# INK-USC/RE-Net

Hardware: AMD Instinct MI355X
Metric: RGCN+GRU encoder triples/s at bs=1024 n_hidden=200 (full training step, both directions) (higher is better)
Workload: dtype f32; 1 GPU; ICEWS18-shaped synthetic stream (seed 999), n_hidden=200, seq_len=10, batch=1024 per GPU, dropout=0.50, fwd+bwd both directions + clip + Adam; parallelism=dp1, global_batch=1024, nodes=99312, edges=288792

## Files before the change

re-net_amd/csrc/gemm.hip:

```cpp
#include <cstdint>
#include <cstdlib>
#include <type_traits>
#include "common.h"

namespace {

constexpr int BM = 128, BN = 128, BK = 32;
constexpr int LDK = BK + 4;
constexpr int LDR = BM + 4;
constexpr int OPBUF = BM * LDK;
constexpr int THREADS = 256;
static_assert(BK * LDR <= OPBUF, "operand buffer too small");

typedef float f32x16 __attribute__((ext_vector_type(16)));

struct GemmArgs {
    const float* A;
    const float* B;
    float* C;
    const float* bias;
    int M, N, K, lda, ldb, ldc;
    float alpha, beta;
    int k_tiles_per_split;
    int split_k;
    float* partial;
    int xcd_order;
};

template <bool CONTIG_K>
__device__ __forceinline__ void load_tile(const float* __restrict__ P, int ld, int rows, int K, int row0,
                                          int k0, int tid, bool vec_ok, float4 (&r)[4]) {
#pragma unroll
    for (int i = 0; i < 4; ++i) {
        const int f = tid + THREADS * i;
        float4 v = make_float4(0.f, 0.f, 0.f, 0.f);
        if constexpr (CONTIG_K) {
            const int row = row0 + (f >> 3), k = k0 + ((f & 7) << 2);
            if (row < rows) {
                const float* p = P + (size_t)row * ld + k;
                if (vec_ok && k + 3 < K) v = *reinterpret_cast<const float4*>(p);
                else {
                    if (k < K) v.x = p[0];
                    if (k + 1 < K) v.y = p[1];
                    if (k + 2 < K) v.z = p[2];
                    if (k + 3 < K) v.w = p[3];
                }
            }
        } else {
            const int k = k0 + (f >> 5), row = row0 + ((f & 31) << 2);
            if (k < K) {
                const float* p = P + (size_t)k * ld + row;
                if (vec_ok && row + 3 < rows) v = *reinterpret_cast<const float4*>(p);
                else {
                    if (row < rows) v.x = p[0];
                    if (row + 1 < rows) v.y = p[1];
                    if (row + 2 < rows) v.z = p[2];
                    if (row + 3 < rows) v.w = p[3];
                }
            }
        }
        r[i] = v;
    }
}

__device__ __forceinline__ float4 shift_tail(float4 v, int d) {
    if (d == 1) return make_float4(v.y, v.z, v.w, 0.f);
    if (d == 2) return make_float4(v.z, v.w, 0.f, 0.f);
    return make_float4(v.w, 0.f, 0.f, 0.f);
}

template <bool CONTIG_K>
__device__ __forceinline__ void load_tile_any(const float* __restrict__ P, int ld, int rows, int K, int row0,
                                              int k0, int tid, bool small, float4 (&r)[4]) {
    if (small) {
        load_tile<CONTIG_K>(P, ld, rows, K, row0, k0, tid, false, r);
        return;
    }
#pragma unroll
    for (int i = 0; i < 4; ++i) {
        const int f = tid + THREADS * i;
        const int c = CONTIG_K ? k0 + ((f & 7) << 2) : row0 + ((f & 31) << 2);
        const int o = CONTIG_K ? row0 + (f >> 3) : k0 + (f >> 5);
        const int C = CONTIG_K ? K : rows;
        const int O = CONTIG_K ? rows : K;
        r[i] = *reinterpret_cast<const float4*>(P + (size_t)min(o, O - 1) * ld + min(c, C - 4));
    }
}

template <bool CONTIG_K>
__device__ __forceinline__ void store_tile(float* __restrict__ S, int rows, int K, int row0, int k0, int tid,
                                           bool small, const float4 (&r)[4]) {
#pragma unroll
    for (int i = 0; i < 4; ++i) {
        const int f = tid + THREADS * i;
        float4 v = r[i];
        if (!small) {
            const int c = CONTIG_K ? k0 + ((f & 7) << 2) : row0 + ((f & 31) << 2);
            const int o = CONTIG_K ? row0 + (f >> 3) : k0 + (f >> 5);
            const int C = CONTIG_K ? K : rows;
            const int O = CONTIG_K ? rows : K;
            if (o >= O || c >= C) v = make_float4(0.f, 0.f, 0.f, 0.f);
            else if (c > C - 4) v = shift_tail(v, c - (C - 4));
        }
        if constexpr (CONTIG_K) *reinterpret_cast<float4*>(&S[(f >> 3) * LDK + ((f & 7) << 2)]) = v;
        else *reinterpret_cast<float4*>(&S[(f >> 5) * LDR + ((f & 31) << 2)]) = v;
    }
}

template <bool CONTIG_K>
__device__ __forceinline__ float4 read_frag(const float* __restrict__ S, int row, int g, int ksel) {
    if constexpr (CONTIG_K) {
        return *reinterpret_cast<const float4*>(&S[row * LDK + 8 * g + 4 * ksel]);
    } else {
        const float* p = S + (8 * g + 4 * ksel) * LDR + row;
        return make_float4(p[0], p[LDR], p[2 * LDR], p[3 * LDR]);
    }
}

template <bool TA, bool TB>
__global__ __launch_bounds__(THREADS) void gemm_f32_generic_kernel(GemmArgs g) {
    __shared__ __attribute__((aligned(16))) float smem[2][2][OPBUF];
    const int tid = threadIdx.x;
    const int lane = tid & 63, wave = tid >> 6;
    const int wm = wave >> 1, wn = wave & 1;
    const int m0 = blockIdx.y * BM, n0 = blockIdx.x * BN;
    const int z = blockIdx.z;
    const int kt0 = z * g.k_tiles_per_split;
    const int kt_total = (g.K + BK - 1) / BK;
    const int kt1 = min(kt_total, kt0 + g.k_tiles_per_split);

    constexpr bool A_CK = !TA;
    constexpr bool B_CK = TB;
    const bool a_vec = ((g.lda & 3) == 0) && ((reinterpret_cast<uintptr_t>(g.A) & 15) == 0);
    const bool b_vec = ((g.ldb & 3) == 0) && ((reinterpret_cast<uintptr_t>(g.B) & 15) == 0);

    f32x16 acc[2][2];
#pragma unroll
    for (int i = 0; i < 2; ++i)
#pragma unroll
        for (int j = 0; j < 2; ++j)
#pragma unroll
            for (int r = 0; r < 16; ++r) acc[i][j][r] = 0.f;

    (void)a_vec; (void)b_vec;
    const bool a_full = (g.K < 4) || (g.M < 4);
    const bool b_full = (g.K < 4) || (g.N < 4);
    float4 ra[4], rb[4];
    if (kt0 < kt1) {
        load_tile_any<A_CK>(g.A, g.lda, g.M, g.K, m0, kt0 * BK, tid, a_full, ra);
        load_tile_any<B_CK>(g.B, g.ldb, g.N, g.K, n0, kt0 * BK, tid, b_full, rb);
        store_tile<A_CK>(smem[0][0], g.M, g.K, m0, kt0 * BK, tid, a_full, ra);
        store_tile<B_CK>(smem[0][1], g.N, g.K, n0, kt0 * BK, tid, b_full, rb);
        if (kt0 + 1 < kt1) {
            load_tile_any<A_CK>(g.A, g.lda, g.M, g.K, m0, (kt0 + 1) * BK, tid, a_full, ra);
            load_tile_any<B_CK>(g.B, g.ldb, g.N, g.K, n0, (kt0 + 1) * BK, tid, b_full, rb);
        }
    }
    __syncthreads();
    const int arow = wm * 64 + (lane & 31);
    const int brow = wn * 64 + (lane & 31);
    const int ksel = lane >> 5;

    for (int kt = kt0; kt < kt1; ++kt) {
        const int cur = (kt - kt0) & 1;
        if (kt + 1 < kt1) {
            store_tile<A_CK>(smem[cur ^ 1][0], g.M, g.K, m0, (kt + 1) * BK, tid, a_full, ra);
            store_tile<B_CK>(smem[cur ^ 1][1], g.N, g.K, n0, (kt + 1) * BK, tid, b_full, rb);
        }
        if (kt + 2 < kt1) {
            load_tile_any<A_CK>(g.A, g.lda, g.M, g.K, m0, (kt + 2) * BK, tid, a_full, ra);
            load_tile_any<B_CK>(g.B, g.ldb, g.N, g.K, n0, (kt + 2) * BK, tid, b_full, rb);
        }
        const float* As = smem[cur][0];
        const float* Bs = smem[cur][1];
#pragma unroll
        for (int kg = 0; kg < BK / 8; ++kg) {
            const float4 a0 = read_frag<A_CK>(As, arow, kg, ksel);
            const float4 a1 = read_frag<A_CK>(As, arow + 32, kg, ksel);
            const float4 b0 = read_frag<B_CK>(Bs, brow, kg, ksel);
            const float4 b1 = read_frag<B_CK>(Bs, brow + 32, kg, ksel);
            acc[0][0] = __builtin_amdgcn_mfma_f32_32x32x2f32(a0.x, b0.x, acc[0][0], 0, 0, 0);
            acc[0][1] = __builtin_amdgcn_mfma_f32_32x32x2f32(a0.x, b1.x, acc[0][1], 0, 0, 0);
            acc[1][0] = __builtin_amdgcn_mfma_f32_32x32x2f32(a1.x, b0.x, acc[1][0], 0, 0, 0);
            acc[1][1] = __builtin_amdgcn_mfma_f32_32x32x2f32(a1.x, b1.x, acc[1][1], 0, 0, 0);
            acc[0][0] = __builtin_amdgcn_mfma_f32_32x32x2f32(a0.y, b0.y, acc[0][0], 0, 0, 0);
            acc[0][1] = __builtin_amdgcn_mfma_f32_32x32x2f32(a0.y, b1.y, acc[0][1], 0, 0, 0);
            acc[1][0] = __builtin_amdgcn_mfma_f32_32x32x2f32(a1.y, b0.y, acc[1][0], 0, 0, 0);
            acc[1][1] = __builtin_amdgcn_mfma_f32_32x32x2f32(a1.y, b1.y, acc[1][1], 0, 0, 0);
            acc[0][0] = __builtin_amdgcn_mfma_f32_32x32x2f32(a0.z, b0.z, acc[0][0], 0, 0, 0);
            acc[0][1] = __builtin_amdgcn_mfma_f32_32x32x2f32(a0.z, b1.z, acc[0][1], 0, 0, 0);
            acc[1][0] = __builtin_amdgcn_mfma_f32_32x32x2f32(a1.z, b0.z, acc[1][0], 0, 0, 0);
            acc[1][1] = __builtin_amdgcn_mfma_f32_32x32x2f32(a1.z, b1.z, acc[1][1], 0, 0, 0);
            acc[0][0] = __builtin_amdgcn_mfma_f32_32x32x2f32(a0.w, b0.w, acc[0][0], 0, 0, 0);
            acc[0][1] = __builtin_amdgcn_mfma_f32_32x32x2f32(a0.w, b1.w, acc[0][1], 0, 0, 0);
            acc[1][0] = __builtin_amdgcn_mfma_f32_32x32x2f32(a1.w, b0.w, acc[1][0], 0, 0, 0);
            acc[1][1] = __builtin_amdgcn_mfma_f32_32x32x2f32(a1.w, b1.w, acc[1][1], 0, 0, 0);
        }
        __syncthreads();
    }

    const bool split = g.split_k > 1;
    float* Cout = split ? g.partial + (size_t)z * g.M * g.N : g.C;
    const int ldo = split ? g.N : g.ldc;
#pragma unroll
    for (int i = 0; i < 2; ++i)
#pragma unroll
        for (int j = 0; j < 2; ++j) {
            const int col = n0 + wn * 64 + j * 32 + (lane & 31);
            if (col >= g.N) continue;
            const float bv = (!split && g.bias) ? g.bias[col] : 0.f;
#pragma unroll
            for (int r = 0; r < 16; ++r) {
                const int row = m0 + wm * 64 + i * 32 + (r & 3) + 8 * (r >> 2) + 4 * ksel;
                if (row < g.M) {
                    float* p = Cout + (size_t)row * ldo + col;
                    if (split) *p = acc[i][j][r];
                    else {
                        float v = g.alpha * acc[i][j][r] + bv;
                        if (g.beta != 0.f) v += g.beta * (*p);
                        *p = v;
                    }
                }
            }
        }
}

typedef uint32_t u32x4 __attribute__((ext_vector_type(4)));

__device__ __forceinline__ void tile_of_block(int nbx, int nby, bool xcd_order, int& bx, int& by, int& bz) {
    bz = blockIdx.z;
    if (!xcd_order) { bx = blockIdx.x; by = blockIdx.y; return; }
    const int nb = nbx * nby;
    int t;
    if (gridDim.z == 1) {
        const int per = nb >> 3;
        const int L = blockIdx.x + nbx * blockIdx.y;
        t = L < 8 * per ? (L & 7) * per + (L >> 3) : L;
    } else {
        const int total = nb * (int)gridDim.z, per3 = total >> 3;
        const int L3 = blockIdx.x + nbx * (blockIdx.y + nby * blockIdx.z);
        const int v = L3 < 8 * per3 ? (L3 & 7) * per3 + (L3 >> 3) : L3;
        bz = v / nb;
        t = v - bz * nb;
    }
    const int ns = min(nbx, nby), nl = max(nbx, nby);
    const int w = min(ns, 8);
    const int p = t / (w * nl), r = t - p * (w * nl);
    const int wp = min(w, ns - p * w);
    const int l = r / wp, sh = p * w + (r - l * wp);
    if (nby <= nbx) { bx = l; by = sh; }
    else { by = l; bx = sh; }
}

template <bool CONTIG_K, int KT>
struct BufLoader {
    static constexpr int NI = KT / 8;
    static constexpr int CPR = KT / 4;
    static constexpr int LDKT = KT + 4;
    __amdgpu_buffer_rsrc_t rs;
    uint32_t off[NI];
    uint32_t kstep;
    int lim[NI];
    int rows, K;

    __device__ __forceinline__ void init(const float* P, int ld, int rows_, int K_, int row0, int tid) {
        rows = rows_; K = K_;
        const uint32_t extent = CONTIG_K ? (uint32_t)(rows - 1) * (uint32_t)ld + (uint32_t)K
                                         : (uint32_t)(K - 1) * (uint32_t)ld + (uint32_t)rows;
        rs = __builtin_amdgcn_make_buffer_rsrc(const_cast<float*>(P), (short)0, (int)(extent * 4u), 0x00020000);
        kstep = CONTIG_K ? (uint32_t)KT * 4u : (uint32_t)KT * (uint32_t)ld * 4u;
#pragma unroll
        for (int i = 0; i < NI; ++i) {
            const int f = tid + THREADS * i;
            if constexpr (CONTIG_K) {
                const int row = row0 + f / CPR, k = (f % CPR) << 2;
                off[i] = ((uint32_t)min(row, rows - 1) * (uint32_t)ld + (uint32_t)k) * 4u;
                lim[i] = k;
            } else {
                const int k = f >> 5, row = row0 + ((f & 31) << 2);
                off[i] = ((uint32_t)k * (uint32_t)ld + (uint32_t)min(row, rows - 1)) * 4u;
                lim[i] = 0;
            }
        }
    }

    __device__ __forceinline__ float4 load(int i, int kt) const {
        const u32x4 v = __builtin_amdgcn_raw_buffer_load_b128(rs, (int)(off[i] + (uint32_t)kt * kstep), 0, 0);
        return make_float4(__uint_as_float(v.x), __uint_as_float(v.y), __uint_as_float(v.z), __uint_as_float(v.w));
    }

    __device__ __forceinline__ float4 fix(int i, int k0, float4 v) const {
        if constexpr (CONTIG_K) {
            const int room = K - k0 - lim[i];
            v.x = room > 0 ? v.x : 0.f;
            v.y = room > 1 ? v.y : 0.f;
            v.z = room > 2 ? v.z : 0.f;
            v.w = room > 3 ? v.w : 0.f;
        }
        return v;
    }

    __device__ __forceinline__ void store(float* __restrict__ S, int i, int tid, float4 v) const {
        const int f = tid + THREADS * i;
        if constexpr (CONTIG_K) *reinterpret_cast<float4*>(&S[(f / CPR) * LDKT + ((f % CPR) << 2)]) = v;
        else *reinterpret_cast<float4*>(&S[(f >> 5) * LDR + ((f & 31) << 2)]) = v;
    }

    static __device__ __forceinline__ float4 frag(const float* __restrict__ S, int row, int g, int ksel) {
        if constexpr (CONTIG_K) {
            return *reinterpret_cast<const float4*>(&S[row * LDKT + 8 * g + 4 * ksel]);
        } else {
            const float* p = S + (8 * g + 4 * ksel) * LDR + row;
            return make_float4(p[0], p[LDR], p[2 * LDR], p[3 * LDR]);
        }
    }
};

template <int I, int N, class F>
__device__ __forceinline__ void static_for(F&& f) {
    if constexpr (I < N) {
        f(std::integral_constant<int, I>{});
        static_for<I + 1, N>(f);
    }
}

__device__ __forceinline__ float f4_get(const float4& v, int t) { return t == 0 ? v.x : t == 1 ? v.y : t == 2 ? v.z : v.w; }

__device__ __forceinline__ void store_acc(const GemmArgs& g, int m0, int n0, int z, int wm, int wn, int lane,
                                          const f32x16 (&acc)[2][2]) {
    const bool split = g.split_k > 1;
    float* Cout = split ? g.partial + (size_t)z * g.M * g.N : g.C;
    const int ldo = split ? g.N : g.ldc;
    const int half = lane >> 5;
    const bool accumulate = !split && g.beta != 0.f;
#pragma unroll
    for (int i = 0; i < 2; ++i)
#pragma unroll
        for (int j = 0; j < 2; ++j) {
            const int col = n0 + wn * 64 + j * 32 + (lane & 31);
            if (col >= g.N) continue;
            const float bv = (!split && g.bias) ? g.bias[col] : 0.f;
            const int row_base = m0 + wm * 64 + i * 32 + 4 * half;
            float old[16];
#pragma unroll
            for (int r = 0; r < 16; ++r) old[r] = 0.f;
            if (accumulate) {
#pragma unroll
                for (int r = 0; r < 16; ++r) {
                    const int row = min(row_base + (r & 3) + 8 * (r >> 2), g.M - 1);
                    old[r] = Cout[(size_t)row * ldo + col];
                }
            }
#pragma unroll
            for (int r = 0; r < 16; ++r) {
                const int row = row_base + (r & 3) + 8 * (r >> 2);
                if (row < g.M) {
                    float* p = Cout + (size_t)row * ldo + col;
                    if (split) *p = acc[i][j][r];
                    else *p = g.alpha * acc[i][j][r] + bv + (accumulate ? g.beta * old[r] : 0.f);
                }
            }
        }
}

#ifndef F32P_NOBAR
#define F32_LOOP_BARRIER() asm volatile("s_waitcnt lgkmcnt(0)\n\ts_barrier" ::: "memory")
#else
#define F32_LOOP_BARRIER() asm volatile("s_waitcnt lgkmcnt(0)" ::: "memory")
#endif

template <bool TA, bool TB, int KT, int WPE>
__global__ __launch_bounds__(THREADS, WPE) void gemm_f32_kernel(GemmArgs g) {
    constexpr bool A_CK = !TA;
    constexpr bool B_CK = TB;
    typedef BufLoader<A_CK, KT> LA;
    typedef BufLoader<B_CK, KT> LB;
    constexpr int NI = KT / 8, NG = KT / 8, NM = 16 * NG;
    constexpr int OPB = (BM * (KT + 4) > KT * LDR) ? BM * (KT + 4) : KT * LDR;
    __shared__ __attribute__((aligned(16))) float smem[2][2][OPB];
    const int tid = threadIdx.x;
    const int lane = tid & 63, wave = tid >> 6;
    const int wm = wave >> 1, wn = wave & 1;
    int bx, by, z;
    tile_of_block(gridDim.x, gridDim.y, g.xcd_order != 0, bx, by, z);
    const int m0 = by * BM, n0 = bx * BN;
    const int kt0 = z * g.k_tiles_per_split;
    const int kt_total = (g.K + KT - 1) / KT;
    const int kt1 = min(kt_total, kt0 + g.k_tiles_per_split);

    f32x16 acc[2][2];
#pragma unroll
    for (int i = 0; i < 2; ++i)
#pragma unroll
        for (int j = 0; j < 2; ++j)
#pragma unroll
            for (int r = 0; r < 16; ++r) acc[i][j][r] = 0.f;

    LA la;
    LB lb;
    la.init(g.A, g.lda, g.M, g.K, m0, tid);
    lb.init(g.B, g.ldb, g.N, g.K, n0, tid);
    float4 ra[NI], rb[NI];
#pragma unroll
    for (int i = 0; i < NI; ++i) { ra[i] = la.load(i, kt0); rb[i] = lb.load(i, kt0); }
#pragma unroll
    for (int i = 0; i < NI; ++i) {
        la.store(smem[0][0], i, tid, la.fix(i, kt0 * KT, ra[i]));
        lb.store(smem[0][1], i, tid, lb.fix(i, kt0 * KT, rb[i]));
    }
#pragma unroll
    for (int i = 0; i < NI; ++i) { ra[i] = la.load(i, kt0 + 1); rb[i] = lb.load(i, kt0 + 1); }
    asm volatile("s_waitcnt lgkmcnt(0)\n\ts_barrier" ::: "memory");

    const int arow = wm * 64 + (lane & 31);
    const int brow = wn * 64 + (lane & 31);
    const int ksel = lane >> 5;

    auto k_tile = [&](int kt, auto fixc) {
        constexpr bool FIX = decltype(fixc)::value;
        const int cur = (kt - kt0) & 1;
        const float* As = smem[cur][0];
        const float* Bs = smem[cur][1];
        float* An = smem[cur ^ 1][0];
        float* Bn = smem[cur ^ 1][1];
        float4 fa[2][2], fb[2][2];
        fa[0][0] = LA::frag(As, arow, 0, ksel);
        fb[0][0] = LB::frag(Bs, brow, 0, ksel);
        fa[0][1] = LA::frag(As, arow + 32, 0, ksel);
        fb[0][1] = LB::frag(Bs, brow + 32, 0, ksel);
        static_for<0, NM>([&](auto mc) {
            constexpr int m = mc.value, grp = m >> 4, t = (m >> 2) & 3, i = (m >> 1) & 1, j = m & 1, fbuf = grp & 1;
            acc[i][j] = __builtin_amdgcn_mfma_f32_32x32x2f32(f4_get(fa[fbuf][i], t), f4_get(fb[fbuf][j], t), acc[i][j],
                                                             0, 0, 0);
            __builtin_amdgcn_sched_barrier(0);
            if constexpr (grp + 1 < NG && (m & 15) < 4) {
                constexpr int q = m & 15;
                if constexpr (q == 0) fa[fbuf ^ 1][0] = LA::frag(As, arow, grp + 1, ksel);
                if constexpr (q == 1) fb[fbuf ^ 1][0] = LB::frag(Bs, brow, grp + 1, ksel);
                if constexpr (q == 2) fa[fbuf ^ 1][1] = LA::frag(As, arow + 32, grp + 1, ksel);
                if constexpr (q == 3) fb[fbuf ^ 1][1] = LB::frag(Bs, brow + 32, grp + 1, ksel);
            }
#ifndef F32P_NOSTAGE
            constexpr int STRIDE = (NM - 6) / (2 * NI);
            if constexpr (m >= 4 && (m - 4) % STRIDE == 0 && (m - 4) / STRIDE < 2 * NI) {
                constexpr int pc = (m - 4) / STRIDE, it = pc >> 1;
                if constexpr ((pc & 1) == 0) la.store(An, it, tid, FIX ? la.fix(it, (kt + 1) * KT, ra[it]) : ra[it]);
                else lb.store(Bn, it, tid, FIX ? lb.fix(it, (kt + 1) * KT, rb[it]) : rb[it]);
            }
            if constexpr (m >= 5 && (m - 5) % STRIDE == 0 && (m - 5) / STRIDE < 2 * NI) {
                constexpr int pc = (m - 5) / STRIDE, it = pc >> 1;
                if constexpr ((pc & 1) == 0) ra[it] = la.load(it, kt + 2);
                else rb[it] = lb.load(it, kt + 2);
            }
#endif
            __builtin_amdgcn_sched_barrier(0);
        });
        F32_LOOP_BARRIER();
    };
    const int kt_plain = min(kt1, kt_total - 2);
    int kt = kt0;
    for (; kt < kt_plain; ++kt) k_tile(kt, std::false_type{});
    for (; kt < kt1; ++kt) k_tile(kt, std::true_type{});
    store_acc(g, m0, n0, z, wm, wn, lane, acc);
}

__global__ __launch_bounds__(256) void splitk_reduce_kernel(const float* __restrict__ partial, int split_k,
                                                            int M, int N, float alpha, float beta,
                                                            const float* __restrict__ bias,
                                                            float* __restrict__ C, int ldc) {
    const size_t total = (size_t)M * N;
    for (size_t i = (size_t)blockIdx.x * blockDim.x + threadIdx.x; i < total;
         i += (size_t)gridDim.x * blockDim.x) {
        const int m = (int)(i / N), n = (int)(i % N);
        float s = 0.f;
        for (int z = 0; z < split_k; ++z) s += partial[(size_t)z * total + i];
        float v = alpha * s + (bias ? bias[n] : 0.f);
        float* p = C + (size_t)m * ldc + n;
        if (beta != 0.f) v += beta * (*p);
        *p = v;
    }
}

template <typename T>
__global__ __launch_bounds__(256) void colsum_kernel(const T* __restrict__ X, int M, int N, int ldx,
                                                     int rows_per_group, float beta, float* __restrict__ out) {
    __shared__ float red[4][64];
    const int lane = threadIdx.x & 63, wave = threadIdx.x >> 6;
    const int n = blockIdx.x * 64 + lane;
    const int g = blockIdx.y;
    const int m0 = g * rows_per_group, m1 = min(M, m0 + rows_per_group);
    float s0 = 0.f, s1 = 0.f, s2 = 0.f, s3 = 0.f;
    if (n < N) {
        int m = m0 + wave;
        for (; m + 12 < m1; m += 16) {
            s0 += (float)X[(size_t)m * ldx + n];
            s1 += (float)X[(size_t)(m + 4) * ldx + n];
            s2 += (float)X[(size_t)(m + 8) * ldx + n];
            s3 += (float)X[(size_t)(m + 12) * ldx + n];
        }
        for (; m < m1; m += 4) s0 += (float)X[(size_t)m * ldx + n];
    }
    red[wave][lane] = (s0 + s1) + (s2 + s3);
    __syncthreads();
    if (wave == 0 && n < N) {
        float r = (red[0][lane] + red[1][lane]) + (red[2][lane] + red[3][lane]);
        float* o = out + (size_t)g * N + n;
        if (beta != 0.f) r += beta * (*o);
        *o = r;
    }
}

__global__ __launch_bounds__(256) void scale_dev_kernel(float* __restrict__ x, size_t n,
                                                        const float* __restrict__ scale, float bound_in,
                                                        float* __restrict__ bound_out) {
    const float f = *scale;
    if (bound_out && blockIdx.x == 0 && threadIdx.x == 0) *bound_out = fabsf(f) * bound_in;
    if (f == 1.f) return;
    const size_t n4 = n >> 2;
    float4* x4 = reinterpret_cast<float4*>(x);
    for (size_t i = (size_t)blockIdx.x * blockDim.x + threadIdx.x; i < n4; i += (size_t)gridDim.x * blockDim.x) {
        float4 v = x4[i];
        x4[i] = make_float4(v.x * f, v.y * f, v.z * f, v.w * f);
    }
    if (blockIdx.x == 0 && threadIdx.x < (n & 3)) x[(n4 << 2) + threadIdx.x] *= f;
}

__global__ __launch_bounds__(256) void scale_dev_bf16_kernel(__bf16* __restrict__ x, size_t n,
                                                             const float* __restrict__ scale) {
    const float f = *scale;
    if (f == 1.f) return;
    for (size_t i = (size_t)blockIdx.x * blockDim.x + threadIdx.x; i < n; i += (size_t)gridDim.x * blockDim.x)
        x[i] = (__bf16)((float)x[i] * f);
}

inline int colsum_groups(int M) { return max(1, min(64, (M + 127) / 128)); }

template <typename T>
int colsum_impl(const T* X, int M, int N, int ldx, float* out, float beta, float* workspace,
                       size_t workspace_bytes, void* stream) {
    if (M < 0 || N <= 0 || ldx < N) return RENET_ERR_BADARG;
    const int G = colsum_groups(M);
    hipStream_t st = (hipStream_t)stream;
    if (G == 1) {
        RENET_LAUNCH((colsum_kernel<T>), dim3((N + 63) / 64, 1), dim3(256), 0, st, X, M, N, ldx, max(M, 1), beta, out);
        RENET_LAUNCH_CHECK();
        return RENET_OK;
    }
    if (workspace_bytes < (size_t)colsum_groups(M) * N * sizeof(float)) return RENET_ERR_WORKSPACE;
    const int rpg = (M + G - 1) / G;
    RENET_LAUNCH((colsum_kernel<T>), dim3((N + 63) / 64, G), dim3(256), 0, st, X, M, N, ldx, rpg, 0.f, workspace);
    RENET_LAUNCH_CHECK();
    RENET_LAUNCH((colsum_kernel<float>), dim3((N + 63) / 64, 1), dim3(256), 0, st, (const float*)workspace, G, N, N, G,
                 beta, out);
    RENET_LAUNCH_CHECK();
    return RENET_OK;
}


bool generic_forced() {
    static const bool v = renet_env_flag("RENET_GEMM_F32_GENERIC", false);
    return v;
}

}

extern "C" {

size_t renet_gemm_workspace(int M, int N, int split_k) {
    return split_k > 1 ? (size_t)split_k * (size_t)M * (size_t)N * sizeof(float) : 0;
}

int renet_gemm_f32(int ta, int tb, int M, int N, int K, float alpha, const float* A, int lda,
                   const float* B, int ldb, float beta, float* C, int ldc, const float* bias,
                   int split_k, float* workspace, size_t workspace_bytes, void* stream) {
    if (M < 0 || N < 0 || K < 0 || lda <= 0 || ldb <= 0 || ldc < N) return RENET_ERR_BADARG;
    if (M == 0 || N == 0) return RENET_OK;
    if (split_k < 1) split_k = 1;
    const int kt_total = (K + BK - 1) / BK;
    if (split_k > kt_total) split_k = max(kt_total, 1);
    if (split_k > 1 && workspace_bytes < renet_gemm_workspace(M, N, split_k)) return RENET_ERR_WORKSPACE;
    GemmArgs g;
    g.A = A; g.B = B; g.C = C; g.bias = bias; g.M = M; g.N = N; g.K = K;
    g.lda = lda; g.ldb = ldb; g.ldc = ldc; g.alpha = alpha; g.beta = beta;
    g.split_k = split_k;
    g.k_tiles_per_split = (kt_total + split_k - 1) / split_k;
    if (g.k_tiles_per_split < 1) g.k_tiles_per_split = 1;
    g.partial = workspace;
    g.xcd_order = renet_gemm_tile_order() != 0;
    hipStream_t st = (hipStream_t)stream;
    const dim3 grid((N + BN - 1) / BN, (M + BM - 1) / BM, split_k);
    const size_t reach_a = ta ? ((size_t)K + 3 * BK) * lda + M : (size_t)M * lda + K + 3 * BK;
    const size_t reach_b = tb ? (size_t)N * ldb + K + 3 * BK : ((size_t)K + 3 * BK) * ldb + N;
    const bool buffered = K >= 1 && reach_a < ((size_t)1 << 30) && reach_b < ((size_t)1 << 30) && !generic_forced();
    if (buffered) {
        constexpr int kt = 32;
        const int ktiles = (K + kt - 1) / kt;
        if (split_k > ktiles) { split_k = max(ktiles, 1); g.split_k = split_k; }
        g.k_tiles_per_split = max(1, (ktiles + split_k - 1) / split_k);
        const dim3 gridb((N + BN - 1) / BN, (M + BM - 1) / BM, split_k);
#define RENET_F32_LAUNCH(KT_, WPE_)                                                                                   \
        do {                                                                                                          \
            if (!ta && !tb) RENET_LAUNCH((gemm_f32_kernel<false, false, KT_, WPE_>), gridb, dim3(THREADS), 0, st, g); \
            else if (!ta && tb) RENET_LAUNCH((gemm_f32_kernel<false, true, KT_, WPE_>), gridb, dim3(THREADS), 0, st, g); \
            else if (ta && !tb) RENET_LAUNCH((gemm_f32_kernel<true, false, KT_, WPE_>), gridb, dim3(THREADS), 0, st, g); \
            else RENET_LAUNCH((gemm_f32_kernel<true, true, KT_, WPE_>), gridb, dim3(THREADS), 0, st, g);              \
        } while (0)
        RENET_F32_LAUNCH(32, 2);
#undef RENET_F32_LAUNCH
    } else {
        g.xcd_order = 0;
        if (!ta && !tb) RENET_LAUNCH((gemm_f32_generic_kernel<false, false>), grid, dim3(THREADS), 0, st, g);
        else if (!ta && tb) RENET_LAUNCH((gemm_f32_generic_kernel<false, true>), grid, dim3(THREADS), 0, st, g);
        else if (ta && !tb) RENET_LAUNCH((gemm_f32_generic_kernel<true, false>), grid, dim3(THREADS), 0, st, g);
        else RENET_LAUNCH((gemm_f32_generic_kernel<true, true>), grid, dim3(THREADS), 0, st, g);
    }
    RENET_LAUNCH_CHECK();
    if (split_k > 1) {
        const size_t total = (size_t)M * N;
        int blocks = (int)min((size_t)2048, (total + 255) / 256);
        RENET_LAUNCH(splitk_reduce_kernel, dim3(blocks), dim3(256), 0, st, workspace, split_k, M, N,
                           alpha, beta, bias, C, ldc);
        RENET_LAUNCH_CHECK();
    }
    return RENET_OK;
}

size_t renet_colsum_workspace(int M, int N) {
    const int G = colsum_groups(M);
    return G > 1 ? (size_t)G * (size_t)N * sizeof(float) : 0;
}

int renet_scale_by_device_scalar(float* x, size_t n, const float* scale, void* stream) {
    if (!x || !scale || (reinterpret_cast<uintptr_t>(x) & 15)) return RENET_ERR_BADARG;
    if (n == 0) return RENET_OK;
    const int blocks = (int)min((size_t)2048, (n / 4 + 255) / 256 + 1);
    RENET_LAUNCH(scale_dev_kernel, dim3(blocks), dim3(256), 0, (hipStream_t)stream, x, n, scale, 0.f, (float*)nullptr);
    RENET_LAUNCH_CHECK();
    return RENET_OK;
}

int renet_scale_by_device_scalar_bound(float* x, size_t n, const float* scale, float bound_in, float* bound_out,
                                       void* stream) {
    if (!x || !scale || !bound_out || (reinterpret_cast<uintptr_t>(x) & 15)) return RENET_ERR_BADARG;
    const int blocks = (int)min((size_t)2048, (n / 4 + 255) / 256 + 1);
    RENET_LAUNCH(scale_dev_kernel, dim3(blocks), dim3(256), 0, (hipStream_t)stream, x, n, scale, bound_in, bound_out);
    RENET_LAUNCH_CHECK();
    return RENET_OK;
}

int renet_colsum(const float* X, int M, int N, int ldx, float* out, float beta, float* workspace,
                 size_t workspace_bytes, void* stream) {
    return colsum_impl<float>(X, M, N, ldx, out, beta, workspace, workspace_bytes, stream);
}

int renet_colsum_bf16(const void* X, int M, int N, int ldx, float* out, float beta, float* workspace,
                      size_t workspace_bytes, void* stream) {
    return colsum_impl<__bf16>((const __bf16*)X, M, N, ldx, out, beta, workspace, workspace_bytes, stream);
}

int renet_scale_bf16_by_device_scalar(void* x, size_t n, const float* scale, void* stream) {
    if (n == 0) return RENET_OK;
    const int blocks = (int)min((size_t)2048, (n + 255) / 256);
    RENET_LAUNCH(scale_dev_bf16_kernel, dim3(blocks), dim3(256), 0, (hipStream_t)stream, (__bf16*)x, n, scale);
    RENET_LAUNCH_CHECK();
    return RENET_OK;
}

}
```

re-net_amd/csrc/rows.hip:

```cpp
#include "common.h"

namespace {

__global__ __launch_bounds__(256) void gather_rows_kernel(const float4* __restrict__ table,
                                                          const int32_t* __restrict__ idx, int n, int CH,
                                                          float4* __restrict__ out) {
    const size_t total = (size_t)n * CH;
    for (size_t i = (size_t)blockIdx.x * blockDim.x + threadIdx.x; i < total;
         i += (size_t)gridDim.x * blockDim.x) {
        const int r = (int)(i / CH), c = (int)(i % CH);
        out[i] = table[(size_t)idx[r] * CH + c];
    }
}

constexpr int kSegWaves = 16, kSegShort = 16, kSegUnr = 8;
__global__ __launch_bounds__(kSegWaves * 64) void segment_add_kernel(const float4* __restrict__ src0,
                                                                     const float4* __restrict__ src1,
                                                                     const int32_t* __restrict__ order,
                                                                     const int32_t* __restrict__ seg_ptr,
                                                                     const int32_t* __restrict__ seg_target,
                                                                     int U, int CH, float4* __restrict__ dst0,
                                                                     float4* __restrict__ dst1) {
    const float4* __restrict__ src = blockIdx.y ? src1 : src0;
    float4* __restrict__ dst = blockIdx.y ? dst1 : dst0;
    __shared__ float4 red[kSegWaves][128];
    const int lane = threadIdx.x & 63;
    const int wave = __builtin_amdgcn_readfirstlane(threadIdx.x >> 6);
    const int nwg = gridDim.x;
    {
        const int u = blockIdx.x + wave * nwg;
        const int k0 = u < U ? seg_ptr[u] : 0, k1 = u < U ? seg_ptr[u + 1] : 0;
        const int len = k1 - k0;
        if (len > 0 && len <= kSegShort) {
            const size_t tgt = (size_t)seg_target[u] * CH;
            for (int ch = lane; ch < CH; ch += 64) {
                float4 s = make_float4(0.f, 0.f, 0.f, 0.f);
                for (int k = k0; k < k1; k += kSegUnr) {
                    float4 v[kSegUnr];
#pragma unroll
                    for (int j = 0; j < kSegUnr; ++j) v[j] = src[(size_t)order[min(k + j, k1 - 1)] * CH + ch];
#pragma unroll
                    for (int j = 0; j < kSegUnr; ++j)
                        if (k + j < k1) s = f4_add(s, v[j]);
                }
                dst[tgt + ch] = f4_add(dst[tgt + ch], s);
            }
        }
    }
    for (int j = 0; j < kSegWaves; ++j) {
        const int u = blockIdx.x + j * nwg;
        if (u >= U) break;
        const int k0 = seg_ptr[u], k1 = seg_ptr[u + 1];
        if (k1 - k0 <= kSegShort) continue;
        const size_t tgt = (size_t)seg_target[u] * CH;
        for (int ch = lane; ch < CH; ch += 64) {
            float4 s = make_float4(0.f, 0.f, 0.f, 0.f);
            for (int k = k0 + wave * kSegUnr; k < k1; k += kSegWaves * kSegUnr) {
                float4 v[kSegUnr];
#pragma unroll
                for (int q = 0; q < kSegUnr; ++q) v[q] = src[(size_t)order[min(k + q, k1 - 1)] * CH + ch];
#pragma unroll
                for (int q = 0; q < kSegUnr; ++q)
                    if (k + q < k1) s = f4_add(s, v[q]);
            }
            red[wave][ch] = s;
        }
        __syncthreads();
        if (wave == 0) {
            for (int ch = lane; ch < CH; ch += 64) {
                float4 r = red[0][ch];
#pragma unroll
                for (int w = 1; w < kSegWaves; ++w) r = f4_add(r, red[w][ch]);
                dst[tgt + ch] = f4_add(dst[tgt + ch], r);
            }
        }
        __syncthreads();
    }
}

}

extern "C" {

int renet_version(void) { return RENET_ABI_VERSION; }

int renet_gather_rows(const float* table, const int32_t* idx, int n, int D, float* out, void* stream) {
    if (n < 0 || D <= 0 || (D & 3)) return RENET_ERR_BADARG;
    if (n == 0) return RENET_OK;
    const int CH = D / 4;
    const size_t total = (size_t)n * CH;
    int blocks = (int)min((size_t)2048, (total + 255) / 256);
    RENET_LAUNCH(gather_rows_kernel, dim3(blocks), dim3(256), 0, (hipStream_t)stream,
                       (const float4*)table, idx, n, CH, (float4*)out);
    RENET_LAUNCH_CHECK();
    return RENET_OK;
}

static int seg_grid(int U) { return U <= 512 ? U : max(512, (U + kSegWaves - 1) / kSegWaves); }

int renet_segment_add(const float* src, const int32_t* order, const int32_t* seg_ptr,
                      const int32_t* seg_target, int U, int D, float* dst, void* stream) {
    if (U < 0 || D <= 0 || (D & 3)) return RENET_ERR_BADARG;
    if (U == 0) return RENET_OK;
    if (D > 512) return RENET_ERR_UNSUPPORTED;
    RENET_LAUNCH(segment_add_kernel, dim3(seg_grid(U)), dim3(kSegWaves * 64), 0,
                       (hipStream_t)stream, (const float4*)src, (const float4*)src, order, seg_ptr, seg_target, U, D / 4,
                       (float4*)dst, (float4*)dst);
    RENET_LAUNCH_CHECK();
    return RENET_OK;
}

int renet_segment_add2(const float* src0, const float* src1, const int32_t* order, const int32_t* seg_ptr,
                       const int32_t* seg_target, int U, int D, float* dst0, float* dst1, void* stream) {
    if (U < 0 || D <= 0 || (D & 3)) return RENET_ERR_BADARG;
    if (U == 0) return RENET_OK;
    if (D > 512) return RENET_ERR_UNSUPPORTED;
    RENET_LAUNCH(segment_add_kernel, dim3(seg_grid(U), 2), dim3(kSegWaves * 64), 0,
                       (hipStream_t)stream, (const float4*)src0, (const float4*)src1, order, seg_ptr, seg_target, U, D / 4,
                       (float4*)dst0, (float4*)dst1);
    RENET_LAUNCH_CHECK();
    return RENET_OK;
}

}
```

Baseline: 391,300 triples/s.

## Restructure segment-add work split and vectorize column-sum kernel

Segment-add is reorganized into two kinds of workgroups in one launch. Some workgroups collect long segments and reduce each with 16 chains across 8 waves. The rest give one wave per short or medium segment, using readlane-broadcast indices, length-specialized unrolled gathers and software-prefetched segment bounds. The column-sum reduction also gains a float4-vectorized variant, used when stride and alignment allow. The aim is to cut load imbalance, index-load latency and per-element scalar loads in the scatter-add and bias-gradient paths, at the cost of more complex code and extra shared-memory atomics for classifying segments.

```diff
diff --git a/re-net_amd/csrc/gemm.hip b/re-net_amd/csrc/gemm.hip
--- a/re-net_amd/csrc/gemm.hip
+++ b/re-net_amd/csrc/gemm.hip
@@ -510,6 +510,70 @@
     }
 }
 
+constexpr int kColsumUnr = 8;
+template <typename T>
+__global__ __launch_bounds__(256) void colsum_vec_kernel(const T* __restrict__ X, int M, int N, int ldx,
+                                                         int rows_per_group, float beta, float* __restrict__ out) {
+    typedef T vec4 __attribute__((ext_vector_type(4)));
+    __shared__ float red[4][4][64];
+    const int lane = threadIdx.x & 63;
+    const int wave = __builtin_amdgcn_readfirstlane(threadIdx.x >> 6);
+    const int a = lane >> 4, n4 = blockIdx.x * 64 + (lane & 15) * 4;
+    const int g = blockIdx.y;
+    const int m0 = g * rows_per_group, m1 = min(M, m0 + rows_per_group);
+    const int b = m0 + wave;
+    const int I = m1 - 12 > b ? (m1 - 12 - b + 15) >> 4 : 0;
+    const int bt = b + 16 * I;
+    float s[4] = {0.f, 0.f, 0.f, 0.f};
+    if (n4 + 3 < N) {
+        const T* col = X + n4;
+        for (int i = 0; i < I; i += kColsumUnr) {
+            vec4 v[kColsumUnr];
+#pragma unroll
+            for (int j = 0; j < kColsumUnr; ++j)
+                v[j] = *reinterpret_cast<const vec4*>(col + (size_t)(b + 4 * a + 16 * min(i + j, I - 1)) * ldx);
+#pragma unroll
+            for (int j = 0; j < kColsumUnr; ++j) {
+                const bool on = i + j < I;
+#pragma unroll
+                for (int c = 0; c < 4; ++c) s[c] = on ? s[c] + (float)v[j][c] : s[c];
+            }
+        }
+        if (a == 0 && bt < m1) {
+            vec4 v[3];
+#pragma unroll
+            for (int j = 0; j < 3; ++j) v[j] = *reinterpret_cast<const vec4*>(col + (size_t)min(bt + 4 * j, m1 - 1) * ldx);
+#pragma unroll
+            for (int j = 0; j < 3; ++j) {
+                const bool on = bt + 4 * j < m1;
+#pragma unroll
+                for (int c = 0; c < 4; ++c) s[c] = on ? s[c] + (float)v[j][c] : s[c];
+            }
+        }
+    } else if (n4 < N) {
+        for (int i = 0; i < I; ++i)
+            for (int c = 0; c < 4; ++c)
+                if (n4 + c < N) s[c] += (float)X[(size_t)(b + 4 * a + 16 * i) * ldx + n4 + c];
+        if (a == 0)
+            for (int m = bt; m < m1; m += 4)
+                for (int c = 0; c < 4; ++c)
+                    if (n4 + c < N) s[c] += (float)X[(size_t)m * ldx + n4 + c];
+    }
+#pragma unroll
+    for (int c = 0; c < 4; ++c) red[wave][a][(lane & 15) * 4 + c] = s[c];
+    __syncthreads();
+    const int n = blockIdx.x * 64 + lane;
+    if (wave == 0 && n < N) {
+        float r[4];
+#pragma unroll
+        for (int w = 0; w < 4; ++w) r[w] = (red[w][0][lane] + red[w][1][lane]) + (red[w][2][lane] + red[w][3][lane]);
+        float t = (r[0] + r[1]) + (r[2] + r[3]);
+        float* o = out + (size_t)g * N + n;
+        if (beta != 0.f) t += beta * (*o);
+        *o = t;
+    }
+}
+
 __global__ __launch_bounds__(256) void scale_dev_kernel(float* __restrict__ x, size_t n,
                                                         const float* __restrict__ scale, float bound_in,
                                                         float* __restrict__ bound_out) {
@@ -536,22 +600,28 @@
 inline int colsum_groups(int M) { return max(1, min(64, (M + 127) / 128)); }
 
 template <typename T>
+void colsum_launch(const T* X, int M, int N, int ldx, int G, int rpg, float beta, float* out, hipStream_t st) {
+    const bool vec = (ldx & 3) == 0 && ((uintptr_t)X & (4 * sizeof(T) - 1)) == 0;
+    if (vec) RENET_LAUNCH((colsum_vec_kernel<T>), dim3((N + 63) / 64, G), dim3(256), 0, st, X, M, N, ldx, rpg, beta, out);
+    else RENET_LAUNCH((colsum_kernel<T>), dim3((N + 63) / 64, G), dim3(256), 0, st, X, M, N, ldx, rpg, beta, out);
+}
+
+template <typename T>
 int colsum_impl(const T* X, int M, int N, int ldx, float* out, float beta, float* workspace,
                        size_t workspace_bytes, void* stream) {
     if (M < 0 || N <= 0 || ldx < N) return RENET_ERR_BADARG;
     const int G = colsum_groups(M);
     hipStream_t st = (hipStream_t)stream;
     if (G == 1) {
-        RENET_LAUNCH((colsum_kernel<T>), dim3((N + 63) / 64, 1), dim3(256), 0, st, X, M, N, ldx, max(M, 1), beta, out);
+        colsum_launch<T>(X, M, N, ldx, 1, max(M, 1), beta, out, st);
         RENET_LAUNCH_CHECK();
         return RENET_OK;
     }
     if (workspace_bytes < (size_t)colsum_groups(M) * N * sizeof(float)) return RENET_ERR_WORKSPACE;
     const int rpg = (M + G - 1) / G;
-    RENET_LAUNCH((colsum_kernel<T>), dim3((N + 63) / 64, G), dim3(256), 0, st, X, M, N, ldx, rpg, 0.f, workspace);
+    colsum_launch<T>(X, M, N, ldx, G, rpg, 0.f, workspace, st);
     RENET_LAUNCH_CHECK();
-    RENET_LAUNCH((colsum_kernel<float>), dim3((N + 63) / 64, 1), dim3(256), 0, st, (const float*)workspace, G, N, N, G,
-                 beta, out);
+    colsum_launch<float>((const float*)workspace, G, N, N, 1, G, beta, out, st);
     RENET_LAUNCH_CHECK();
     return RENET_OK;
 }
diff --git a/re-net_amd/csrc/rows.hip b/re-net_amd/csrc/rows.hip
--- a/re-net_amd/csrc/rows.hip
+++ b/re-net_amd/csrc/rows.hip
@@ -13,68 +13,154 @@
     }
 }
 
-constexpr int kSegWaves = 16, kSegShort = 16, kSegUnr = 8;
-__global__ __launch_bounds__(kSegWaves * 64) void segment_add_kernel(const float4* __restrict__ src0,
-                                                                     const float4* __restrict__ src1,
-                                                                     const int32_t* __restrict__ order,
-                                                                     const int32_t* __restrict__ seg_ptr,
-                                                                     const int32_t* __restrict__ seg_target,
-                                                                     int U, int CH, float4* __restrict__ dst0,
-                                                                     float4* __restrict__ dst1) {
+constexpr int kSegShort = 16, kSegUnr = 8, kSegChains = 16, kSegMedium = kSegChains * kSegUnr, kSegWaves = 8;
+constexpr int kSegThreads = kSegWaves * 64, kSegMaxCH = 128;
+
+__device__ __forceinline__ float4 seg_sel(bool c, float4 a, float4 b) {
+    return make_float4(c ? a.x : b.x, c ? a.y : b.y, c ? a.z : b.z, c ? a.w : b.w);
+}
+
+template <int NR>
+__device__ __forceinline__ void seg_short_rows(const float4* __restrict__ src, float4* __restrict__ dst, int idx,
+                                               size_t tgt, int len, int CH, int lane) {
+    for (int c0 = 0; c0 < CH; c0 += 64) {
+        const int ch = c0 + lane, chc = min(ch, CH - 1);
+        float4 v[NR];
+#pragma unroll
+        for (int j = 0; j < NR; ++j) v[j] = src[(size_t)__builtin_amdgcn_readlane(idx, j) * CH + chc];
+        const float4 old = dst[tgt + chc];
+        float4 s = make_float4(0.f, 0.f, 0.f, 0.f);
+#pragma unroll
+        for (int j = 0; j < NR; ++j) s = seg_sel(j < len, f4_add(s, v[j]), s);
+        if (ch < CH) dst[tgt + ch] = f4_add(old, s);
+    }
+}
+
+__device__ __forceinline__ void seg_medium_rows(const float4* __restrict__ src, float4* __restrict__ dst,
+                                                const int32_t* __restrict__ order, int idx0, int k0, size_t tgt, int len,
+                                                int CH, int lane) {
+    const int idx1 = order[min(k0 + 64 + lane, k0 + len - 1)];
+    for (int c0 = 0; c0 < CH; c0 += 64) {
+        const int ch = c0 + lane, chc = min(ch, CH - 1);
+        const float4 old = dst[tgt + chc];
+        float4 r = make_float4(0.f, 0.f, 0.f, 0.f);
+        const float4 zero = make_float4(0.f, 0.f, 0.f, 0.f);
+        int b = 0;
+#pragma unroll 1
+        for (; 2 * kSegUnr * b < len; ++b) {
+            const int idx = b < 4 ? idx0 : idx1, l0 = (2 * kSegUnr * b) & 63;
+            float4 c[2], v[2 * kSegUnr];
+            c[0] = c[1] = zero;
+#pragma unroll
+            for (int q = 0; q < 2 * kSegUnr; ++q) v[q] = src[(size_t)__builtin_amdgcn_readlane(idx, l0 + q) * CH + chc];
+#pragma unroll
+            for (int q = 0; q < 2 * kSegUnr; ++q)
+                c[q / kSegUnr] = seg_sel(2 * kSegUnr * b + q < len, f4_add(c[q / kSegUnr], v[q]), c[q / kSegUnr]);
+            r = seg_sel(b == 0, c[0], f4_add(r, c[0]));
+            r = f4_add(r, c[1]);
+        }
+        for (; b < kSegChains / 2; ++b) r = f4_add(f4_add(r, zero), zero);
+        if (ch < CH) dst[tgt + ch] = f4_add(old, r);
+    }
+}
+
+__global__ __launch_bounds__(kSegThreads) __attribute__((amdgpu_waves_per_eu(2, 4))) void segment_add_kernel(
+    const float4* __restrict__ src0, const float4* __restrict__ src1, const int32_t* __restrict__ order,
+    const int32_t* __restrict__ seg_ptr, const int32_t* __restrict__ seg_target, int U, int CH, int n_long_wg,
+    float4* __restrict__ dst0, float4* __restrict__ dst1) {
     const float4* __restrict__ src = blockIdx.y ? src1 : src0;
     float4* __restrict__ dst = blockIdx.y ? dst1 : dst0;
-    __shared__ float4 red[kSegWaves][128];
-    const int lane = threadIdx.x & 63;
-    const int wave = __builtin_amdgcn_readfirstlane(threadIdx.x >> 6);
-    const int nwg = gridDim.x;
-    {
-        const int u = blockIdx.x + wave * nwg;
-        const int k0 = u < U ? seg_ptr[u] : 0, k1 = u < U ? seg_ptr[u + 1] : 0;
-        const int len = k1 - k0;
-        if (len > 0 && len <= kSegShort) {
-            const size_t tgt = (size_t)seg_target[u] * CH;
-            for (int ch = lane; ch < CH; ch += 64) {
-                float4 s = make_float4(0.f, 0.f, 0.f, 0.f);
-                for (int k = k0; k < k1; k += kSegUnr) {
-                    float4 v[kSegUnr];
-#pragma unroll
-                    for (int j = 0; j < kSegUnr; ++j) v[j] = src[(size_t)order[min(k + j, k1 - 1)] * CH + ch];
-#pragma unroll
-                    for (int j = 0; j < kSegUnr; ++j)
-                        if (k + j < k1) s = f4_add(s, v[j]);
+    __shared__ float4 red[kSegChains][kSegMaxCH];
+    __shared__ int list[kSegThreads];
+    __shared__ int cnt;
+    const int tid = threadIdx.x, lane = tid & 63;
+    const int wave = __builtin_amdgcn_readfirstlane(tid >> 6);
+
+    if ((int)blockIdx.x >= n_long_wg) {
+        const int gw = (blockIdx.x - n_long_wg) * kSegWaves + wave;
+        const int nw = (gridDim.x - n_long_wg) * kSegWaves;
+        const int R = seg_ptr[U];
+        if (R <= 0) return;
+        auto bound = [&](long long u, int& k0, int& k1) {
+            const int uc = (int)min(u, (long long)U - 1);
+            const int a = seg_ptr[uc], b = seg_ptr[uc + 1];
+            k0 = u < U ? a : 0;
+            k1 = u < U ? b : 0;
+        };
+        auto entries = [&](long long u, int k0, int len, int& idx, int& tgt) {
+            idx = order[min(k0 + min(lane, max(len - 1, 0)), R - 1)];
+            tgt = seg_target[(int)min(u, (long long)U - 1)];
+        };
+        long long u = gw;
+        int k0, k1, idx, tgt, nk0, nk1;
+        bound(u, k0, k1);
+        entries(u, k0, k1 - k0, idx, tgt);
+        bound(u + nw, nk0, nk1);
+        while (u < U) {
+            const int len = k1 - k0, nlen = nk1 - nk0;
+            int nidx, ntgt, nnk0, nnk1;
+            entries(u + nw, nk0, nlen, nidx, ntgt);
+            bound(u + 2ll * nw, nnk0, nnk1);
+            if (len > 0 && len <= kSegMedium) {
+                const size_t t = (size_t)tgt * CH;
+                if (len == 1) seg_short_rows<1>(src, dst, idx, t, len, CH, lane);
+                else if (len == 2) seg_short_rows<2>(src, dst, idx, t, len, CH, lane);
+                else if (len <= 4) seg_short_rows<4>(src, dst, idx, t, len, CH, lane);
+                else if (len <= 8) seg_short_rows<8>(src, dst, idx, t, len, CH, lane);
+                else if (len <= kSegShort) seg_short_rows<16>(src, dst, idx, t, len, CH, lane);
+                else seg_medium_rows(src, dst, order, idx, k0, t, len, CH, lane);
+            }
+            u += nw;
+            k0 = nk0, k1 = nk1, idx = nidx, tgt = ntgt, nk0 = nnk0, nk1 = nnk1;
+        }
+        return;
+    }
+
+    float* __restrict__ dstf = reinterpret_cast<float*>(dst);
+    const long long G = n_long_wg;
+    bool first = true;
+    for (long long base = 0; blockIdx.x + base * G < U; base += kSegThreads) {
+        __syncthreads();
+        if (tid == 0) cnt = 0;
+        __syncthreads();
+        const long long u = blockIdx.x + (base + tid) * G;
+        if (u < U && seg_ptr[u + 1] - seg_ptr[u] > kSegMedium) list[atomicAdd(&cnt, 1)] = (int)u;
+        __syncthreads();
+        const int n = cnt;
+        for (int i = 0; i < n; ++i) {
+            const int us = __builtin_amdgcn_readfirstlane(list[i]);
+            const int k0 = seg_ptr[us], k1 = seg_ptr[us + 1];
+            const size_t tgt = (size_t)seg_target[us] * CH * 4;
+            const float old = tid < 4 * CH ? dstf[tgt + tid] : 0.f;
+            if (!first) __syncthreads();
+            first = false;
+            for (int c0 = 0; c0 < CH; c0 += 64) {
+                const int ch = c0 + lane, chc = min(ch, CH - 1);
+                float4 s[2];
+                s[0] = s[1] = make_float4(0.f, 0.f, 0.f, 0.f);
+                int kb = k0 + 2 * kSegUnr * wave;
+                int idx = order[min(kb + (lane & 15), k1 - 1)];
+                for (; kb < k1; kb += kSegChains * kSegUnr) {
+                    const int idx_next = order[min(kb + kSegChains * kSegUnr + (lane & 15), k1 - 1)];
+                    float4 v[2 * kSegUnr];
+#pragma unroll
+                    for (int q = 0; q < 2 * kSegUnr; ++q) v[q] = src[(size_t)__builtin_amdgcn_readlane(idx, q) * CH + chc];
+#pragma unroll
+                    for (int q = 0; q < 2 * kSegUnr; ++q)
+                        s[q / kSegUnr] = seg_sel(kb + q < k1, f4_add(s[q / kSegUnr], v[q]), s[q / kSegUnr]);
+                    idx = idx_next;
                 }
-                dst[tgt + ch] = f4_add(dst[tgt + ch], s);
+                if (ch < CH) red[2 * wave][ch] = s[0], red[2 * wave + 1][ch] = s[1];
+            }
+            __syncthreads();
+            if (tid < 4 * CH) {
+                const float* redf = reinterpret_cast<const float*>(&red[0][0]);
+                float r = redf[tid];
+#pragma unroll
+                for (int w = 1; w < kSegChains; ++w) r += redf[w * 4 * kSegMaxCH + tid];
+                dstf[tgt + tid] = old + r;
             }
         }
-    }
-    for (int j = 0; j < kSegWaves; ++j) {
-        const int u = blockIdx.x + j * nwg;
-        if (u >= U) break;
-        const int k0 = seg_ptr[u], k1 = seg_ptr[u + 1];
-        if (k1 - k0 <= kSegShort) continue;
-        const size_t tgt = (size_t)seg_target[u] * CH;
-        for (int ch = lane; ch < CH; ch += 64) {
-            float4 s = make_float4(0.f, 0.f, 0.f, 0.f);
-            for (int k = k0 + wave * kSegUnr; k < k1; k += kSegWaves * kSegUnr) {
-                float4 v[kSegUnr];
-#pragma unroll
-                for (int q = 0; q < kSegUnr; ++q) v[q] = src[(size_t)order[min(k + q, k1 - 1)] * CH + ch];
-#pragma unroll
-                for (int q = 0; q < kSegUnr; ++q)
-                    if (k + q < k1) s = f4_add(s, v[q]);
-            }
-            red[wave][ch] = s;
-        }
-        __syncthreads();
-        if (wave == 0) {
-            for (int ch = lane; ch < CH; ch += 64) {
-                float4 r = red[0][ch];
-#pragma unroll
-                for (int w = 1; w < kSegWaves; ++w) r = f4_add(r, red[w][ch]);
-                dst[tgt + ch] = f4_add(dst[tgt + ch], r);
-            }
-        }
-        __syncthreads();
     }
 }
 
@@ -96,30 +182,30 @@
     return RENET_OK;
 }
 
-static int seg_grid(int U) { return U <= 512 ? U : max(512, (U + kSegWaves - 1) / kSegWaves); }
+static int seg_wave_wgs(int U) { return (max(min(U, 2048), (U + 7) / 8) + kSegWaves - 1) / kSegWaves; }
+static int seg_long_wgs(int U) { return min(U, 256); }
+
+static int segment_add_impl(const float* src0, const float* src1, const int32_t* order, const int32_t* seg_ptr,
+                            const int32_t* seg_target, int U, int D, float* dst0, float* dst1, int pairs, void* stream) {
+    if (U < 0 || D <= 0 || (D & 3)) return RENET_ERR_BADARG;
+    if (U == 0) return RENET_OK;
+    if (D > 4 * kSegMaxCH) return RENET_ERR_UNSUPPORTED;
+    const int G = seg_long_wgs(U);
+    RENET_LAUNCH(segment_add_kernel, dim3(G + seg_wave_wgs(U), pairs), dim3(kSegThreads), 0, (hipStream_t)stream,
+                 (const float4*)src0, (const float4*)src1, order, seg_ptr, seg_target, U, D / 4, G, (float4*)dst0,
+                 (float4*)dst1);
+    RENET_LAUNCH_CHECK();
+    return RENET_OK;
+}
 
 int renet_segment_add(const float* src, const int32_t* order, const int32_t* seg_ptr,
                       const int32_t* seg_target, int U, int D, float* dst, void* stream) {
-    if (U < 0 || D <= 0 || (D & 3)) return RENET_ERR_BADARG;
-    if (U == 0) return RENET_OK;
-    if (D > 512) return RENET_ERR_UNSUPPORTED;
-    RENET_LAUNCH(segment_add_kernel, dim3(seg_grid(U)), dim3(kSegWaves * 64), 0,
-                       (hipStream_t)stream, (const float4*)src, (const float4*)src, order, seg_ptr, seg_target, U, D / 4,
-                       (float4*)dst, (float4*)dst);
-    RENET_LAUNCH_CHECK();
-    return RENET_OK;
+    return segment_add_impl(src, src, order, seg_ptr, seg_target, U, D, dst, dst, 1, stream);
 }
 
 int renet_segment_add2(const float* src0, const float* src1, const int32_t* order, const int32_t* seg_ptr,
                        const int32_t* seg_target, int U, int D, float* dst0, float* dst1, void* stream) {
-    if (U < 0 || D <= 0 || (D & 3)) return RENET_ERR_BADARG;
-    if (U == 0) return RENET_OK;
-    if (D > 512) return RENET_ERR_UNSUPPORTED;
-    RENET_LAUNCH(segment_add_kernel, dim3(seg_grid(U), 2), dim3(kSegWaves * 64), 0,
-                       (hipStream_t)stream, (const float4*)src0, (const float4*)src1, order, seg_ptr, seg_target, U, D / 4,
-                       (float4*)dst0, (float4*)dst1);
-    RENET_LAUNCH_CHECK();
-    return RENET_OK;
-}
-
-}
+    return segment_add_impl(src0, src1, order, seg_ptr, seg_target, U, D, dst0, dst1, 2, stream);
+}
+
+}
```

Measured after the change: 390,800 triples/s. No clear change (-0.1%).
